# nianticlabs/simplerecon

Measured on AMD Instinct MI355X. Metric: depth frames/sec (640x480, 7 src views, 64 planes), higher is better.
Workload: dtype f32

## Files before the change

### include/simplerecon_hip.h

```cpp
#ifndef SIMPLERECON_HIP_H_
#define SIMPLERECON_HIP_H_

#include <stddef.h>
#include <stdint.h>

#ifdef __cplusplus
extern "C" {
#endif

#define SR_OK 0
#define SR_ERR_INVALID_ARGUMENT 1
#define SR_ERR_UNSUPPORTED 2
#define SR_ERR_WORKSPACE_TOO_SMALL 3
#define SR_ERR_HIP_BASE 1000

enum {
  SR_OPT_MLP_SPLIT = 0, SR_OPT_WINO_SPLIT, SR_OPT_WINO_XCD, SR_OPT_WINO_NT, SR_OPT_WINO_KSPLIT, SR_OPT_CONV_WINO,
  SR_OPT_CONV_TILE, SR_OPT_CONV_KSPLIT, SR_OPT_PW_NT, SR_OPT_PW_KS, SR_OPT_PT_CFG, SR_OPT_PT_KS, SR_OPT_DOT_LDS,
  SR_OPT_DOT_LDS_G, SR_OPT_DOT_LDS_CULL, SR_OPT_DOT_LDS_CAP, SR_OPT_UPSAMPLE_QUAD, SR_OPT_POOL_STREAM,
  SR_OPT_MLP_TILE,
  SR_OPT_COUNT
};
int sr_option_count(void);
const char* sr_option_name(int id);
// ... 128 lines not shown
                              int64_t out_batch_stride, int out_pix_stride, int B, int H, int W, int Cin,
                              int Cout, int ksize, int stride, float leaky_slope, void* workspace,
                              size_t workspace_bytes, void* stream);

size_t sr_wino_packed_weight_floats(int Cout, int Cin);
int sr_wino_pack_weights(const float* weight, int Cout, int Cin, float* packed, void* stream);
int sr_conv_prefers_wino(int B, int H, int W, int Cin, int Cout, int ksize, int stride);
int sr_conv3x3_wino_nhwc_fwd(const float* in, int64_t in_batch_stride, int in_pix_stride,
                             const float* packed_u, const float* bias, const float* residual,
                             int64_t res_batch_stride, int res_pix_stride, float* out,
                             int64_t out_batch_stride, int out_pix_stride, int B, int H, int W, int Cin,
                             int Cout, float leaky_slope, void* stream);

size_t sr_wino4_packed_weight_floats(int Cout, int Cin);
int sr_wino4_pack_weights(const float* weight, int Cout, int Cin, float* packed, void* stream);
int sr_conv_prefers_wino4(int B, int H, int W, int Cin, int Cout, int mode);
int sr_conv3x3_wino4_nhwc_fwd(const float* in, int64_t in_batch_stride, int in_pix_stride, const float* packed_u,
                              const float* bias, const float* residual, int64_t res_batch_stride, int res_pix_stride,
                              float* out, int64_t out_batch_stride, int out_pix_stride, int B, int H, int W, int Cin,
                              int Cout, float leaky_slope, void* stream);

int sr_conv3x3_wino4_variant_nhwc_fwd(const float* in, int64_t in_batch_stride, int in_pix_stride, const float* packed_u,
                                      const float* bias, const float* residual, int64_t res_batch_stride,
                                      int res_pix_stride, float* out, int64_t out_batch_stride, int out_pix_stride, int B,
                                      int H, int W, int Cin, int Cout, float leaky_slope, int variant, void* stream);

int sr_wino_splitk_factor(int B, int H, int W, int Cin, int Cout);
size_t sr_wino_splitk_workspace_bytes(int B, int H, int W, int Cin, int Cout);
int sr_conv3x3_wino_splitk_nhwc_fwd(const float* in, int64_t in_batch_stride, int in_pix_stride,
                                    const float* packed_u, const float* bias, const float* residual,
                                    int64_t res_batch_stride, int res_pix_stride, float* out,
                                    int64_t out_batch_stride, int out_pix_stride, int B, int H, int W, int Cin,
                                    int Cout, float leaky_slope, void* workspace, size_t workspace_bytes,
                                    void* stream);

int sr_wino_conv_plan(int B, int H, int W, int Cin, int Cout, int allow_split, int* nt, int* ks);

int sr_last_launch(char* name, int name_capacity, double* executed_flops);

int sr_upsample2x_nhwc_fwd(const float* in, int64_t in_batch_stride, int in_pix_stride, float* out,
                           int64_t out_batch_stride, int out_pix_stride, int B, int H, int W, int C,
                           void* stream);

int sr_exp_fwd(const float* in, float* out, int64_t n, void* stream);


size_t sr_stem_packed_weight_floats(int Cout);
int sr_stem_pack_weights(const float* weight, int Cout, float* packed, void* stream);

int sr_stem7x7_fwd(const float* in, int64_t in_batch_stride, int64_t in_chan_stride, int64_t in_row_stride,
                   int64_t in_col_stride, const float* packed_weight, const float* scale, const float* shift,
                   float leaky_slope, float* out, int64_t out_batch_stride, int out_pix_stride, int B, int H, int W,
                   int Cout, void* stream);

int sr_maxblurpool_nhwc_fwd(const float* in, int64_t in_batch_stride, int in_pix_stride, float* out,
                            int64_t out_batch_stride, int out_pix_stride, int B, int H, int W, int C, void* stream);

size_t sr_instance_norm_workspace_bytes(int B, int H, int W, int C);
int sr_instance_norm_nhwc_fwd(const float* in, int64_t in_batch_stride, int in_pix_stride, float* out,
                              int64_t out_batch_stride, int out_pix_stride, int B, int H, int W, int C, float eps,
                              float leaky_slope, void* workspace, size_t workspace_bytes, void* stream);

int sr_instance_norm_stats_nhwc(const float* in, int64_t in_batch_stride, int in_pix_stride, int B, int H, int W, int C,
                                float eps, float* stats, void* workspace, size_t workspace_bytes, void* stream);

size_t sr_conv1x1_stats_workspace_bytes(int B, int H, int W, int Cout);
int sr_conv1x1_stats_nhwc_fwd(const float* in, int64_t in_batch_stride, int in_pix_stride, const float* weight,
                              const float* bias, float* out, int64_t out_batch_stride, int out_pix_stride, int B, int H,
                              int W, int Cin, int Cout, float eps, float* stats, void* workspace, size_t workspace_bytes,
                              void* stream);

size_t sr_conv3x3_c16_packed_weight_floats(int Cout, int Cin);
int sr_conv3x3_c16_pack_weights(const float* weight, int Cout, int Cin, float* packed, void* stream);
int sr_conv3x3_c16_nhwc_fwd(const float* in, int64_t in_batch_stride, int in_pix_stride, const float* in_stats,
                            float in_leaky_slope, const float* packed_weight, const float* bias, float* out,
                            int64_t out_batch_stride, int out_pix_stride, int B, int H, int W, int Cin, int Cout,
                            int replicate, float leaky_slope, void* stream);

int sr_tsdf_integrate_fwd(void* tsdf_values, void* tsdf_weights, const void* voxel_coords, int X, int Y, int Z,
                          float origin_x, float origin_y, float origin_z, float voxel_size, const void* depth,
                          const uint8_t* depth_mask, const void* K, const void* T, int B, int H, int W,
                          float min_depth, float max_depth, float depth_range, float truncation, float maxW,
                          void* stream);

size_t sr_mesh_count_scratch_bytes(int X, int Y, int Z);
size_t sr_mesh_list_scratch_bytes(int64_t active);
int sr_mesh_count(const void* tsdf_values, int X, int Y, int Z, float level, void* count_scratch,
                  size_t count_scratch_bytes, int64_t* totals, void* stream);
int sr_mesh_emit(const void* tsdf_values, int X, int Y, int Z, float level, float origin_x, float origin_y, float origin_z,
                 float scale, const void* count_scratch, size_t count_scratch_bytes, void* list_scratch,
                 size_t list_scratch_bytes, int64_t active, int64_t num_vertices, int64_t num_faces, float* vertices,
                 float* normals, int* faces, void* stream);

#define SR_PC_FRAME_FLOATS 36
int sr_pc_consistency(const float* depth, const float* frame_consts, int N, int h, int w, int ref_begin, int ref_count,
                      float z_thresh, float* points, int* counts, void* stream);
int sr_pc_voxel_keys(const float* points, int64_t M, double min_x, double min_y, double min_z, double voxel_size,
                     int64_t* keys, void* stream);
int sr_pc_voxel_mean(const float* points, const uint8_t* colors, int64_t M, const int64_t* order,
                     const int64_t* seg_start, int64_t S, float* out_points, uint8_t* out_colors, void* stream);

#define SR_LOSS_MAX_SOURCES 15
size_t sr_normals_workspace_bytes(int B, int h, int w);
int sr_normals_fwd(const float* depth, const float* invK, int B, int h, int w, float* normals, void* scratch,
                   size_t scratch_bytes, void* stream);
int sr_normals_bwd(const float* grad_normals, const float* depth, const float* invK, int B, int h, int w,
// ... 323 lines not shown
```

### simplerecon_amd/_lib.py

```python
import contextlib
import ctypes as C
import os

import torch

_HERE = os.path.dirname(os.path.abspath(__file__))
LIB_PATH = os.environ.get("SR_HIP_LIBRARY") or os.path.join(_HERE, "libsimplerecon_hip.so")
ABI_VERSION = 4

_lib = None

_p = C.c_void_p
_i = C.c_int
_i64 = C.c_int64
_f = C.c_float
_sz = C.c_size_t

SIGNATURES = {
    "sr_abi_version": (_i, []),
    "sr_option_count": (_i, []),
    "sr_option_name": (C.c_char_p, [_i]),
    "sr_option_id": (_i, [C.c_char_p]),
    "sr_option_get": (_i, [_i, C.POINTER(C.c_int)]),
    "sr_option_set": (_i, [_i, _i, C.POINTER(C.c_int)]),
# ... 71 lines not shown
    "sr_act_bwd": (_i, [_p, _p, _p, _i64, _f, _p]),
    "sr_act_bwd_bias_workspace_bytes": (_sz, [_i64, _i]),
    "sr_act_bwd_bias_nhwc": (_i, [_p, _p, _p, _p, _i64, _i, _f, _p, _sz, _p]),
    "sr_zero_stuff2x_nhwc": (_i, [_p, _i64, _i, _p, _i, _i, _i, _i, _i, _i, _p]),
    "sr_upsample2x_bwd_nhwc": (_i, [_p, _i64, _i, _p, _i64, _i, _i, _i, _i, _i, _p]),
    "sr_conv_flip_transpose_weights": (_i, [_p, _i, _i, _i, _p, _p]),
    "sr_mul_fwd": (_i, [_p, _p, _p, _i64, _p]),
    "sr_norm_workspace_bytes": (_sz, [_i, _i, _i, _i]),
    "sr_norm_stats_nhwc": (_i, [_p, _i64, _i, _i, _i, _i, _i, _p, _p, _p, _sz, _p]),
    "sr_norm_act_fwd_nhwc": (_i, [_p, _i64, _i, _p, _p, _f, _p, _p, _f, _i, _p, _i64, _i, _i, _i, _i, _p]),
    "sr_norm_act_bwd_nhwc": (_i, [_p, _i64, _i, _p, _i64, _i, _p, _p, _f, _p, _p, _f, _i, _i, _p, _i64, _i, _p, _p,
                                  _i, _i, _i, _p, _sz, _p]),
    "sr_rowsum_nhwc": (_i, [_p, _i64, _i, _p, _i64, _i, _i, _i, _i, _f, _p, _p, _sz, _p]),
    "sr_maxblurpool_bwd_workspace_bytes": (_sz, [_i, _i, _i, _i]),
    "sr_maxblurpool_bwd_nhwc": (_i, [_p, _i64, _i, _p, _i64, _i, _p, _i64, _i, _i, _i, _i, _i, _p, _sz, _p]),
    "sr_replicate_pad_nhwc_fwd": (_i, [_p, _i64, _i, _p, _i, _i, _i, _i, _i, _p]),
    "sr_replicate_pad_nhwc_bwd": (_i, [_p, _p, _i, _i, _i, _i, _i, _p]),
    "sr_im2col7x7s2_nhwc": (_i, [_p, _i64, _i64, _i64, _i64, _p, _i, _i, _i, _i, _p]),
    "sr_dwconv3x3_bwd_workspace_bytes": (_sz, [_i, _i, _i, _i]),
    "sr_dwconv3x3_bwd_nhwc": (_i, [_p, _i64, _i, _p, _i64, _i, _p, _p, _p, _i, _i, _i, _i, _i, _i, _i, _i, _i, _p, _sz,
                                   _p]),
    "sr_scale_bwd_nhwc": (_i, [_p, _i64, _i, _p, _p, _f, _p, _i, _i, _i, _p]),
    "sr_small_linear_fwd": (_i, [_p, _p, _p, _p, _p, _i, _i, _i, _f, _p]),
    "sr_small_linear_bwd": (_i, [_p, _p, _p, _p, _p, _p, _p, _i, _i, _i, _f, _p]),
    "sr_act_in_bwd": (_i, [_p, _p, _p, _i64, _f, _p]),
    "sr_add_act_fwd": (_i, [_p, _p, _p, _p, _i64, _f, _p]),
    "sr_conv_wgrad_padded_workspace_bytes": (_sz, [_i, _i, _i, _i, _i, _i]),
    "sr_conv_wgrad_padded_nhwc": (_i, [_p, _i64, _i, _p, _i64, _i, _p, _i, _i, _i, _i, _i, _i, _i, _i, _i, _i, _i, _p,
                                       _sz, _p]),
    "sr_conv_splitk_workspace_bytes": (_sz, [_i, _i, _i, _i, _i, _i, _i]),
    "sr_conv2d_splitk_nhwc_fwd": (_i, [_p, _i64, _i, _p, _p, _p, _i64, _i, _p, _i64, _i, _i, _i, _i, _i, _i, _i, _i,
                                       _f, _p, _sz, _p]),
    "sr_wino_packed_weight_floats": (_sz, [_i, _i]),
    "sr_wino_pack_weights": (_i, [_p, _i, _i, _p, _p]),
    "sr_conv_prefers_wino": (_i, [_i, _i, _i, _i, _i, _i, _i]),
    "sr_wino_splitk_factor": (_i, [_i, _i, _i, _i, _i]),
    "sr_wino_splitk_workspace_bytes": (_sz, [_i, _i, _i, _i, _i]),
    "sr_conv3x3_wino_splitk_nhwc_fwd": (_i, [_p, _i64, _i, _p, _p, _p, _i64, _i, _p, _i64, _i, _i, _i, _i, _i, _i, _f,
                                             _p, _sz, _p]),
    "sr_wino_conv_plan": (_i, [_i, _i, _i, _i, _i, _i, _p, _p]),
    "sr_last_launch": (_i, [_p, _i, _p]),
    "sr_conv3x3_wino_nhwc_fwd": (_i, [_p, _i64, _i, _p, _p, _p, _i64, _i, _p, _i64, _i, _i, _i, _i, _i, _i, _f, _p]),
    "sr_wino4_packed_weight_floats": (_sz, [_i, _i]),
    "sr_wino4_pack_weights": (_i, [_p, _i, _i, _p, _p]),
    "sr_conv_prefers_wino4": (_i, [_i, _i, _i, _i, _i, _i]),
    "sr_conv3x3_wino4_nhwc_fwd": (_i, [_p, _i64, _i, _p, _p, _p, _i64, _i, _p, _i64, _i, _i, _i, _i, _i, _i, _f, _p]),
    "sr_conv3x3_wino4_variant_nhwc_fwd": (_i, [_p, _i64, _i, _p, _p, _p, _i64, _i, _p, _i64, _i, _i, _i, _i, _i, _i, _f, _i,
                                               _p]),
    "sr_upsample2x_nhwc_fwd": (_i, [_p, _i64, _i, _p, _i64, _i, _i, _i, _i, _i, _p]),
    "sr_exp_fwd": (_i, [_p, _p, _i64, _p]),
    "sr_stem_packed_weight_floats": (_sz, [_i]),
    "sr_stem_pack_weights": (_i, [_p, _i, _p, _p]),
    "sr_stem7x7_fwd": (_i, [_p, _i64, _i64, _i64, _i64, _p, _p, _p, _f, _p, _i64, _i, _i, _i, _i, _i, _p]),
    "sr_maxblurpool_nhwc_fwd": (_i, [_p, _i64, _i, _p, _i64, _i, _i, _i, _i, _i, _p]),
    "sr_instance_norm_workspace_bytes": (_sz, [_i, _i, _i, _i]),
    "sr_instance_norm_nhwc_fwd": (_i, [_p, _i64, _i, _p, _i64, _i, _i, _i, _i, _i, _f, _f, _p, _sz, _p]),
    "sr_instance_norm_stats_nhwc": (_i, [_p, _i64, _i, _i, _i, _i, _i, _f, _p, _p, _sz, _p]),
    "sr_conv1x1_stats_workspace_bytes": (_sz, [_i, _i, _i, _i]),
    "sr_conv1x1_stats_nhwc_fwd": (_i, [_p, _i64, _i, _p, _p, _p, _i64, _i, _i, _i, _i, _i, _i, _f, _p, _p, _sz, _p]),
    "sr_conv3x3_c16_packed_weight_floats": (_sz, [_i, _i]),
    "sr_conv3x3_c16_pack_weights": (_i, [_p, _i, _i, _p, _p]),
    "sr_conv3x3_c16_nhwc_fwd": (_i, [_p, _i64, _i, _p, _f, _p, _p, _p, _i64, _i, _i, _i, _i, _i, _i, _i, _f, _p]),
    "sr_tsdf_integrate_fwd": (_i, [_p, _p, _p, _i, _i, _i, _f, _f, _f, _f, _p, _p, _p, _p, _i, _i, _i,
                                   _f, _f, _f, _f, _f, _p]),
    "sr_mesh_count_scratch_bytes": (_sz, [_i, _i, _i]),
    "sr_mesh_list_scratch_bytes": (_sz, [_i64]),
    "sr_mesh_count": (_i, [_p, _i, _i, _i, _f, _p, _sz, _p, _p]),
    "sr_mesh_emit": (_i, [_p, _i, _i, _i, _f, _f, _f, _f, _f, _p, _sz, _p, _sz, _i64, _i64, _i64, _p, _p, _p, _p]),
    "sr_pc_consistency": (_i, [_p, _p, _i, _i, _i, _i, _i, _f, _p, _p, _p]),
    "sr_pc_voxel_keys": (_i, [_p, _i64, C.c_double, C.c_double, C.c_double, C.c_double, _p, _p]),
    "sr_pc_voxel_mean": (_i, [_p, _p, _i64, _p, _p, _i64, _p, _p, _p]),
    "sr_normals_workspace_bytes": (_sz, [_i, _i, _i]),
    "sr_normals_fwd": (_i, [_p, _p, _i, _i, _i, _p, _p, _sz, _p]),
    "sr_normals_bwd": (_i, [_p, _p, _p, _i, _i, _i, _p, _p, _sz, _p]),
    "sr_normals_loss_workspace_bytes": (_sz, [_i, _i, _i]),
    "sr_normals_loss_fwd": (_i, [_p, _p, _i, _i, _i, _p, _p, _sz, _p]),
    "sr_normals_loss_bwd": (_i, [_p, _p, _p, _p, _i, _i, _i, _p, _p]),
    "sr_grad_loss_workspace_bytes": (_sz, [_i, _i, _i]),
    "sr_grad_loss_fwd": (_i, [_p, _p, _i, _i, _i, _p, _p, _sz, _p]),
    "sr_grad_loss_bwd": (_i, [_p, _p, _p, _p, _i, _i, _i, _p, _p, _sz, _p]),
    "sr_mv_loss_workspace_bytes": (_sz, [_i, _i, _i, _i]),
    "sr_mv_loss_fwd": (_i, [_p, _p, _p, _p, _p, _p, _p, _i, _i, _i, _i, _f, _p, _p, _p, _p, _sz, _p]),
    "sr_mv_loss_bwd": (_i, [_p, _p, _p, _p, _p, _p, _p, _p, _p, _i, _i, _i, _i, _f, _p, _p]),
    "sr_depth_terms_workspace_bytes": (_sz, [_i, _i, _i]),
    "sr_depth_terms_fwd": (_i, [_p, _p, _p, _p, _p, _i, _i, _p, _i, _i, _p, _i, _i, _i, _i, _i, _f, _i, _p, _p, _sz,
                                _p]),
    "sr_depth_terms_bwd": (_i, [_p, _p, _p, _p, _p, _p, _p, _i, _i, _p, _i, _i, _p, _i, _i, _i, _i, _i, _f, _i, _p, _p,
                                _p, _p, _p, _p]),
    "sr_depth_metrics_workspace_bytes": (_sz, [_i, _i, _i]),
    "sr_depth_metrics": (_i, [_p, _p, _p, _f, _i, _i, _i, _i, _i, _i, _i, _p, _p, _p, _p, _sz, _p]),
    "sr_depth_metrics_gather": (_i, [_p, _i, _i, _i, _i, _i, _i, _p, _p]),
    "sr_nn_grid_plan": (_i, [_i64, _p, _i64, _p, _p, _p]),
    "sr_nn_keys": (_i, [_p, _i64, C.c_double, C.c_double, C.c_double, C.c_double, _i, _i, _i, _p, _p]),
    "sr_nn_build": (_i, [_p, _i64, _p, _p, _i64, _p, _p, _p]),
    "sr_nn_query": (_i, [_p, _i64, _p, _p, _i64, _p, _i64, C.c_double, C.c_double, C.c_double, C.c_double, _i, _i, _i,
                         _p, _p, _p, _p]),
    "sr_sample_surface_workspace_bytes": (_sz, [_i64]),
    "sr_sample_surface_cdf": (_i, [_p, _i64, _p, _i64, _p, _p, _sz, _p]),
    "sr_sample_surface": (_i, [_p, _i64, _p, _i64, _p, _i64, C.c_uint64, _p, _p, _p]),
    "sr_mesh_metrics_workspace_bytes": (_sz, [_i64, _i64]),
    "sr_mesh_metrics": (_i, [_p, _i64, _p, _i64, _f, _p, _p, _sz, _p]),
    "sr_stsdf_touch": (_i, [_p, _i, _i, _i, _p, C.c_double, C.c_double, _p, _p]),
    "sr_stsdf_block_masks": (_i, [_p, _p, _i64, _i64, _p, _p]),
    "sr_stsdf_integrate": (_i, [_p, _i64, _p, _p, _p, _i64, _p, _p, _p, _i, _i, _i, _f, _f, _p]),
    "sr_stsdf_mesh_count": (_i, [_p, _i64, _p, _p, _i64, _p, _p]),
    "sr_stsdf_mesh_emit": (_i, [_p, _i64, _p, _p, _i64, _f, _p, _i64, _i64, _p, _p, _p, _p, _p]),
# ... 221 lines not shown
```

### simplerecon_amd/csrc/sr_matching.hip

```cpp
#include "sr_common.h"

typedef float v16f __attribute__((ext_vector_type(16)));
#define SR_MFMA(a, b, c) __builtin_amdgcn_mfma_f32_32x32x2f32((a), (b), (c), 0, 0, 0)

#define SR_STEM_T 16
#define SR_STEM_PR 37
#define SR_STEM_PW 37
#define SR_STEM_STEPS 74
#define SR_STEM_WFLOATS (SR_STEM_STEPS * 128)
#define SR_STEM_PFLOATS (3 * SR_STEM_PR * SR_STEM_PW)

struct SrStemParams {
  const float* in; int64_t sb, sc, sy, sx;
  const float* wp;
  const float* scale; const float* shift;
  float slope;
  float* out; int64_t out_sb; int out_sp;
  int H, W, Ho, Wo, tiles_x, tiles_y, total;
};

__global__ void sr_stem_pack_kernel(const float* __restrict__ w , float* __restrict__ packed) {
  for (int idx = blockIdx.x * blockDim.x + threadIdx.x; idx < SR_STEM_WFLOATS; idx += gridDim.x * blockDim.x) {
    const int step = idx >> 7, r = idx & 127;
    const int half = r >> 6, col = (r & 63) >> 1, nt = r & 1;
    const int tap = 2 * step + half;
    const int co = nt * 32 + col;
    packed[idx] = tap < 147 ? w[co * 147 + tap] : 0.f;
  }
}

__host__ __device__ constexpr int sr_stem_tap_offset(int k) {
  return k >= 147 ? 0 : ((k / 49) * SR_STEM_PR + (k % 49) / 7) * SR_STEM_PW + (k % 7);
}

__global__ __launch_bounds__(256, 2) void sr_stem_kernel(SrStemParams p) {
  __shared__ __attribute__((aligned(16))) float wl[SR_STEM_WFLOATS];
  __shared__ float patch[SR_STEM_PFLOATS];
  const int lane = threadIdx.x & 63, wave = threadIdx.x >> 6;
  const int i = lane & 31, half = lane >> 5;

  for (int e = threadIdx.x; e < SR_STEM_WFLOATS / 4; e += 256)
    reinterpret_cast<float4*>(wl)[e] = reinterpret_cast<const float4*>(p.wp)[e];

  int abase[2];
#pragma unroll
  for (int m = 0; m < 2; ++m) abase[m] = (2 * (4 * wave + 2 * m + (i >> 4))) * SR_STEM_PW + 2 * (i & 15);
  const float2* wl2 = reinterpret_cast<const float2*>(wl) + half * 32 + i;

  float sc[2], sh[2];
#pragma unroll
  for (int n = 0; n < 2; ++n) {
    sc[n] = p.scale ? p.scale[n * 32 + i] : 1.f;
    sh[n] = p.shift ? p.shift[n * 32 + i] : 0.f;
  }

  constexpr int PF = (SR_STEM_PFLOATS + 255) / 256;
  float pf[PF];
  auto fetch = [&](int tile) {
    const int tx = tile % p.tiles_x, ty = (tile / p.tiles_x) % p.tiles_y, b = tile / (p.tiles_x * p.tiles_y);
    const float* __restrict__ img = p.in + (int64_t)b * p.sb;
#pragma unroll
    for (int it = 0; it < PF; ++it) {
      const int e = threadIdx.x + it * 256;
      const int c = e / (SR_STEM_PR * SR_STEM_PW), rem = e - c * (SR_STEM_PR * SR_STEM_PW);
      const int r = rem / SR_STEM_PW, x = rem - r * SR_STEM_PW;
      const int gy = 2 * ty * SR_STEM_T - 3 + r, gx = 2 * tx * SR_STEM_T - 3 + x;
      const bool ok = (e < SR_STEM_PFLOATS) & (gy >= 0) & (gy < p.H) & (gx >= 0) & (gx < p.W);
      const int64_t off = ok ? c * p.sc + gy * p.sy + gx * p.sx : 0;
      const float v = img[off];
      pf[it] = ok ? v : 0.f;
    }
  };
  auto stash = [&]() {
#pragma unroll
    for (int it = 0; it < PF; ++it) {
      const int e = threadIdx.x + it * 256;
      if (e < SR_STEM_PFLOATS) patch[e] = pf[it];
    }
  };
  if ((int)blockIdx.x < p.total) fetch(blockIdx.x);
  stash();
  __syncthreads();

  for (int tile = blockIdx.x; tile < p.total; tile += gridDim.x) {
    const int tx = tile % p.tiles_x, ty = (tile / p.tiles_x) % p.tiles_y, b = tile / (p.tiles_x * p.tiles_y);
    const int oy0 = ty * SR_STEM_T, ox0 = tx * SR_STEM_T;
    const int next = tile + gridDim.x;
    if (next < p.total) fetch(next);
    __builtin_amdgcn_sched_barrier(0);

    v16f acc[2][2];
#pragma unroll
    for (int m = 0; m < 2; ++m)
#pragma unroll
      for (int n = 0; n < 2; ++n)
#pragma unroll
        for (int r = 0; r < 16; ++r) acc[m][n][r] = 0.f;

#pragma unroll
    for (int step = 0; step < SR_STEM_STEPS; ++step) {
      constexpr int dummy = 0; (void)dummy;
      const int o0 = sr_stem_tap_offset(2 * step), o1 = sr_stem_tap_offset(2 * step + 1);
      const int oa = (o1 == o0 + 1) ? o0 + half : (half ? o1 : o0);
      const float a0 = patch[abase[0] + oa], a1 = patch[abase[1] + oa];
      const float2 w = wl2[step * 64];
      acc[0][0] = SR_MFMA(a0, w.x, acc[0][0]);
      acc[1][0] = SR_MFMA(a1, w.x, acc[1][0]);
      acc[0][1] = SR_MFMA(a0, w.y, acc[0][1]);
      acc[1][1] = SR_MFMA(a1, w.y, acc[1][1]);
    }
    __builtin_amdgcn_sched_barrier(0);
    __syncthreads();
    if (next < p.total) stash();
    __syncthreads();

    float* __restrict__ ob = p.out + (int64_t)b * p.out_sb;
#pragma unroll
    for (int m = 0; m < 2; ++m)
#pragma unroll
      for (int r = 0; r < 16; ++r) {
        const int mrow = (r & 3) + 8 * (r >> 2) + 4 * half;
        const int oy = oy0 + 4 * wave + 2 * m + (mrow >> 4), ox = ox0 + (mrow & 15);
        if (oy < p.Ho && ox < p.Wo) {
          float* o = ob + ((int64_t)oy * p.Wo + ox) * p.out_sp + i;
#pragma unroll
          for (int n = 0; n < 2; ++n) {
            float v = acc[m][n][r] * sc[n] + sh[n];
            if (p.slope >= 0.f) v = v >= 0.f ? v : v * p.slope;
            o[n * 32] = v;
          }
        }
      }
  }
}

__device__ __forceinline__ int sr_reflect(int i, int n) { return i < 0 ? -i : (i >= n ? 2 * n - 2 - i : i); }
__device__ __forceinline__ float sr_nanmax(float a, float b) { return (a > b || a != a) ? a : b; }
__device__ __forceinline__ float4 sr_max4(float4 a, float4 b) {
  return make_float4(sr_nanmax(a.x, b.x), sr_nanmax(a.y, b.y), sr_nanmax(a.z, b.z), sr_nanmax(a.w, b.w));
}
__device__ __forceinline__ float4 sr_axpy4(float s, float4 a, float4 acc) {
  return make_float4(acc.x + s * a.x, acc.y + s * a.y, acc.z + s * a.z, acc.w + s * a.w);
}

__device__ __forceinline__ float4 sr_ld4(const float* p) { return *reinterpret_cast<const float4*>(p); }

__device__ __forceinline__ float4 sr_maxblur_generic(const float* __restrict__ ib, int in_sp, int W, int Hm, int Wm,
                                                     int oy, int ox, int c4) {
  const float f[4] = {0.125f, 0.375f, 0.375f, 0.125f};
  float4 acc = make_float4(0.f, 0.f, 0.f, 0.f);
  for (int i = 0; i < 4; ++i) {
    const int my = sr_reflect(2 * oy - 1 + i, Hm);
    float4 row = make_float4(0.f, 0.f, 0.f, 0.f);
    for (int j = 0; j < 4; ++j) {
      const int mx = sr_reflect(2 * ox - 1 + j, Wm);
      const float* q = ib + ((int64_t)my * W + mx) * in_sp + 4 * c4;
      row = sr_axpy4(f[j], sr_max4(sr_max4(sr_ld4(q), sr_ld4(q + in_sp)),
                                   sr_max4(sr_ld4(q + (int64_t)W * in_sp), sr_ld4(q + (int64_t)W * in_sp + in_sp))), row);
    }
    acc = sr_axpy4(f[i], row, acc);
  }
  return acc;
}

__global__ __launch_bounds__(256) void sr_maxblurpool_kernel(const float* __restrict__ in, int64_t in_sb, int in_sp,
                                                             float* __restrict__ out, int64_t out_sb, int out_sp,
                                                             int H, int W, int Ho, int Wo, int C4, int xcd_order) {
  constexpr int BW = 2;
  constexpr int WC = 2 * BW + 3;
  const int Hm = H - 1, Wm = W - 1;
  const int bx = (Wo + BW - 1) / BW, by = (Ho + 1) / 2;
  const int64_t total = (int64_t)bx * by * C4;
  const float f[4] = {0.125f, 0.375f, 0.375f, 0.125f};
  unsigned bxi = blockIdx.x, byi = blockIdx.y;
  if (xcd_order) {
    const unsigned T = gridDim.x * gridDim.y, L = blockIdx.y * gridDim.x + blockIdx.x;
    const unsigned Lp = (L & 7u) * (T >> 3) + (L >> 3);
    byi = Lp / gridDim.x;
    bxi = Lp - byi * gridDim.x;
  }
  const float* __restrict__ ib = in + (int64_t)byi * in_sb;
  float* __restrict__ ob = out + (int64_t)byi * out_sb;
  for (int64_t idx = (int64_t)bxi * blockDim.x + threadIdx.x; idx < total; idx += (int64_t)gridDim.x * blockDim.x) {
    const int c4 = (int)(idx % C4);
    const int blk = (int)(idx / C4);
    const int oy0 = 2 * (blk / bx), ox0 = BW * (blk % bx);
// ... 535 lines not shown

extern "C" size_t sr_conv3x3_c16_packed_weight_floats(int Cout, int Cin) {
  if (Cout <= 0 || Cout > 16 || Cin <= 0 || (Cin % 32)) return 0;
  return (size_t)(Cin / 32) * 9 * 2 * 64 * 4;
}

extern "C" int sr_conv3x3_c16_pack_weights(const float* weight, int Cout, int Cin, float* packed, void* stream_) {
  if (!weight || !packed) return SR_ERR_INVALID_ARGUMENT;
  if (Cout <= 0 || Cout > 16 || Cin <= 0 || (Cin % 32)) return SR_ERR_UNSUPPORTED;
  hipLaunchKernelGGL(sr_t16_pack_kernel, dim3(64), dim3(256), 0, (hipStream_t)stream_, weight, packed, Cout, Cin);
  return sr_hip_rc(hipGetLastError());
}

extern "C" int sr_conv3x3_c16_nhwc_fwd(const float* in, int64_t in_batch_stride, int in_pix_stride,
                                       const float* in_stats, float in_leaky_slope, const float* packed_weight,
                                       const float* bias, float* out, int64_t out_batch_stride, int out_pix_stride,
                                       int B, int H, int W, int Cin, int Cout, int replicate, float leaky_slope,
                                       void* stream_) {
  if (B < 0 || H <= 0 || W <= 0 || Cin <= 0 || Cout <= 0) return SR_ERR_INVALID_ARGUMENT;
  if (B == 0) return SR_OK;
  if (!in || !packed_weight || !out) return SR_ERR_INVALID_ARGUMENT;
  if (Cout > 16 || (Cin % 32) || (in_pix_stride % 4) || (in_batch_stride % 4) || ((uintptr_t)in & 15) ||
      (in_stats && ((uintptr_t)in_stats & 15)))
    return SR_ERR_UNSUPPORTED;
  SrT16Params p;
  p.in = in; p.in_sb = in_batch_stride; p.in_sp = in_pix_stride;
  p.stats = in_stats; p.in_slope = in_leaky_slope;
  p.wp = packed_weight; p.bias = bias;
  p.out = out; p.out_sb = out_batch_stride; p.out_sp = out_pix_stride;
  p.H = H; p.W = W; p.Cin = Cin; p.Cout = Cout; p.replicate = replicate;
  p.tiles_x = (W + 15) / 16; p.tiles_y = (H + 7) / 8;
  p.total = p.tiles_x * p.tiles_y * B;
  p.out_slope = leaky_slope;
  int blocks = 3 * sr_cus();
  if (blocks > p.total) blocks = p.total;
  const bool norm = in_stats != nullptr, act = in_leaky_slope >= 0.f;
  sr_note_launch({SR_K_T16, 0, 0, 0, 0, 0, 0, (int64_t)p.total * ((SR_T16_HH - 2) * (SR_T16_HW - 2)), 16, (int64_t)Cin * 9});
  if (norm && act) hipLaunchKernelGGL((sr_t16_kernel<true, true>), dim3(blocks), dim3(256), 0, (hipStream_t)stream_, p);
  else if (norm) hipLaunchKernelGGL((sr_t16_kernel<true, false>), dim3(blocks), dim3(256), 0, (hipStream_t)stream_, p);
  else if (act) hipLaunchKernelGGL((sr_t16_kernel<false, true>), dim3(blocks), dim3(256), 0, (hipStream_t)stream_, p);
  else hipLaunchKernelGGL((sr_t16_kernel<false, false>), dim3(blocks), dim3(256), 0, (hipStream_t)stream_, p);
  return sr_hip_rc(hipGetLastError());
}

extern "C" size_t sr_stem_packed_weight_floats(int Cout) { return Cout == 64 ? (size_t)SR_STEM_WFLOATS : 0; }

extern "C" int sr_stem_pack_weights(const float* weight, int Cout, float* packed, void* stream_) {
  if (!weight || !packed) return SR_ERR_INVALID_ARGUMENT;
  if (Cout != 64) return SR_ERR_UNSUPPORTED;
  hipLaunchKernelGGL(sr_stem_pack_kernel, dim3(42), dim3(256), 0, (hipStream_t)stream_, weight, packed);
  return sr_hip_rc(hipGetLastError());
}

extern "C" int sr_stem7x7_fwd(const float* in, int64_t in_batch_stride, int64_t in_chan_stride, int64_t in_row_stride,
                              int64_t in_col_stride, const float* packed_weight, const float* scale,
                              const float* shift, float leaky_slope, float* out, int64_t out_batch_stride,
                              int out_pix_stride, int B, int H, int W, int Cout, void* stream_) {
  if (B < 0 || H <= 0 || W <= 0) return SR_ERR_INVALID_ARGUMENT;
  if (Cout != 64) return SR_ERR_UNSUPPORTED;
  if (B == 0) return SR_OK;
  if (!in || !packed_weight || !out) return SR_ERR_INVALID_ARGUMENT;
  SrStemParams p;
  p.in = in; p.sb = in_batch_stride; p.sc = in_chan_stride; p.sy = in_row_stride; p.sx = in_col_stride;
  p.wp = packed_weight; p.scale = scale; p.shift = shift; p.slope = leaky_slope;
  p.out = out; p.out_sb = out_batch_stride; p.out_sp = out_pix_stride;
  p.H = H; p.W = W;
  p.Ho = (H + 6 - 7) / 2 + 1; p.Wo = (W + 6 - 7) / 2 + 1;
  p.tiles_x = (p.Wo + SR_STEM_T - 1) / SR_STEM_T; p.tiles_y = (p.Ho + SR_STEM_T - 1) / SR_STEM_T;
  p.total = p.tiles_x * p.tiles_y * B;
  int blocks = 2 * sr_cus();
  if (blocks > p.total) blocks = p.total;
  sr_note_launch({SR_K_STEM, 0, 0, 0, 0, 0, 0, (int64_t)p.total * (SR_STEM_T * SR_STEM_T), 64, 2 * SR_STEM_STEPS});
  hipLaunchKernelGGL(sr_stem_kernel, dim3(blocks), dim3(256), 0, (hipStream_t)stream_, p);
  return sr_hip_rc(hipGetLastError());
}

extern "C" int sr_maxblurpool_nhwc_fwd(const float* in, int64_t in_batch_stride, int in_pix_stride, float* out,
                                       int64_t out_batch_stride, int out_pix_stride, int B, int H, int W, int C,
                                       void* stream_) {
  if (B < 0 || H < 4 || W < 4 || C <= 0) return SR_ERR_INVALID_ARGUMENT;
  if (B == 0) return SR_OK;
  if (!in || !out) return SR_ERR_INVALID_ARGUMENT;
  if ((C % 4) || (in_pix_stride % 4) || (out_pix_stride % 4) || (in_batch_stride % 4) || (out_batch_stride % 4) ||
      ((uintptr_t)in & 15) || ((uintptr_t)out & 15))
    return SR_ERR_UNSUPPORTED;
  const int Ho = (H - 2) / 2 + 1, Wo = (W - 2) / 2 + 1;
  if (sr_opt(SR_OPT_POOL_STREAM) && H >= 16 && W >= 16 && B <= 65535) {
    SrPoolStreamParams p;
    p.in = in; p.in_sb = in_batch_stride; p.in_sp = in_pix_stride;
    p.out = out; p.out_sb = out_batch_stride; p.out_sp = out_pix_stride;
    p.H = H; p.W = W; p.Ho = Ho; p.Wo = Wo; p.C4 = C / 4;
    p.oy_lo = 1; p.oy_hi = (H - 4) / 2; p.ox_lo = 1; p.ox_hi = (W - 4) / 2;
    const int rows = p.oy_hi - p.oy_lo + 1, cols = p.ox_hi - p.ox_lo + 1;
    p.col_blocks = (cols + 1) / 2;
    p.col_groups = (int)(((int64_t)p.col_blocks * p.C4 + 255) / 256);
    const int slots = 2 * sr_cus(), per_band = B * p.col_groups;
    int best_bands = 1;
    double best = -1.0;
    for (int nb = 1; nb <= (rows >= 8 ? rows / 8 : 1); ++nb) {
      const int br = (rows + nb - 1) / nb, real = (rows + br - 1) / br;
      const int64_t wgs = (int64_t)real * per_band;
      const int64_t rounds = (wgs + slots - 1) / slots;
      if (rounds > 10 && best >= 0.0) break;
      const double eff = (double)wgs / (double)(rounds * slots) * (2.0 * br) / (2.0 * br + 3.0);
      if (eff > best + 1e-9) { best = eff; best_bands = real; }
    }
    p.band_rows = (rows + best_bands - 1) / best_bands;
    p.bands = (rows + p.band_rows - 1) / p.band_rows;
    p.stream_wgs = p.bands * p.col_groups;
    p.frame_rows_top = p.oy_lo; p.frame_rows_bottom = Ho - 1 - p.oy_hi;
    p.frame_cols_left = p.ox_lo; p.frame_cols_right = Wo - 1 - p.ox_hi;
    const int64_t frame = ((int64_t)(p.frame_rows_top + p.frame_rows_bottom) * Wo +
                           (int64_t)rows * (p.frame_cols_left + p.frame_cols_right)) * p.C4;
    int frame_wgs = (int)((frame + 255) / 256 < 1024 ? (frame + 255) / 256 : 1024);
    hipLaunchKernelGGL(sr_maxblurpool_stream_kernel, dim3(p.stream_wgs + frame_wgs, B), dim3(256), 0, (hipStream_t)stream_, p);
    return sr_hip_rc(hipGetLastError());
  }
  const int64_t total = (int64_t)((Ho + 1) / 2) * ((Wo + 1) / 2) * (C / 4);
  const int blocks = (int)((total + 255) / 256 < 8192 ? (total + 255) / 256 : 8192);
  const int xcd = ((int64_t)blocks * 256 >= total) && (((int64_t)blocks * B) % 8 == 0);
  hipLaunchKernelGGL(sr_maxblurpool_kernel, dim3(blocks, B), dim3(256), 0, (hipStream_t)stream_, in, in_batch_stride,
                     in_pix_stride, out, out_batch_stride, out_pix_stride, H, W, Ho, Wo, C / 4, xcd);
  return sr_hip_rc(hipGetLastError());
}

static void sr_inorm_chunks(int B, int HW, int* chunks, int* chunk_pix) {
  int want = (8 * sr_cus() + B - 1) / B;
// ... 102 lines not shown
```

Baseline: 329.2.

## Add lean stem 7x7 kernel with prefetched patches and buffer loads

Adds a new path for the 7x7 stem conv that walks tiles persistently. It prefetches the next tile's input patch into registers through buffer loads while the MFMA loop runs on the current tile. Precomputed per-thread offsets, interior-tile fast paths and templated activation/scale variants cut address arithmetic and bounds checks. Bounds-checked buffer stores handle edge tiles. It becomes the default when the strides fit 32-bit buffer ranges, at the cost of more registers and a more complex kernel.

```diff
diff --git a/include/simplerecon_hip.h b/include/simplerecon_hip.h
--- a/include/simplerecon_hip.h
+++ b/include/simplerecon_hip.h
@@ -204,6 +204,11 @@
                    int64_t in_col_stride, const float* packed_weight, const float* scale, const float* shift,
                    float leaky_slope, float* out, int64_t out_batch_stride, int out_pix_stride, int B, int H, int W,
                    int Cout, void* stream);
+
+int sr_stem7x7_variant_fwd(const float* in, int64_t in_batch_stride, int64_t in_chan_stride, int64_t in_row_stride,
+                           int64_t in_col_stride, const float* packed_weight, const float* scale, const float* shift,
+                           float leaky_slope, float* out, int64_t out_batch_stride, int out_pix_stride, int B, int H, int W,
+                           int Cout, int variant, void* stream);
 
 int sr_maxblurpool_nhwc_fwd(const float* in, int64_t in_batch_stride, int in_pix_stride, float* out,
                             int64_t out_batch_stride, int out_pix_stride, int B, int H, int W, int C, void* stream);
diff --git a/simplerecon_amd/_lib.py b/simplerecon_amd/_lib.py
--- a/simplerecon_amd/_lib.py
+++ b/simplerecon_amd/_lib.py
@@ -147,6 +147,7 @@
     "sr_stem_packed_weight_floats": (_sz, [_i]),
     "sr_stem_pack_weights": (_i, [_p, _i, _p, _p]),
     "sr_stem7x7_fwd": (_i, [_p, _i64, _i64, _i64, _i64, _p, _p, _p, _f, _p, _i64, _i, _i, _i, _i, _i, _p]),
+    "sr_stem7x7_variant_fwd": (_i, [_p, _i64, _i64, _i64, _i64, _p, _p, _p, _f, _p, _i64, _i, _i, _i, _i, _i, _i, _p]),
     "sr_maxblurpool_nhwc_fwd": (_i, [_p, _i64, _i, _p, _i64, _i, _i, _i, _i, _i, _p]),
     "sr_instance_norm_workspace_bytes": (_sz, [_i, _i, _i, _i]),
     "sr_instance_norm_nhwc_fwd": (_i, [_p, _i64, _i, _p, _i64, _i, _i, _i, _i, _i, _f, _f, _p, _sz, _p]),
diff --git a/simplerecon_amd/csrc/sr_matching.hip b/simplerecon_amd/csrc/sr_matching.hip
--- a/simplerecon_amd/csrc/sr_matching.hip
+++ b/simplerecon_amd/csrc/sr_matching.hip
@@ -1,4 +1,8 @@
+#include <type_traits>
+
 #include "sr_common.h"
+#include "sr_buffer.h"
+#include "sr_view.h"
 
 typedef float v16f __attribute__((ext_vector_type(16)));
 #define SR_MFMA(a, b, c) __builtin_amdgcn_mfma_f32_32x32x2f32((a), (b), (c), 0, 0, 0)
@@ -17,6 +21,7 @@
   float slope;
   float* out; int64_t out_sb; int out_sp;
   int H, W, Ho, Wo, tiles_x, tiles_y, total;
+  int64_t in_span, out_span;
 };
 
 __global__ void sr_stem_pack_kernel(const float* __restrict__ w , float* __restrict__ packed) {
@@ -33,9 +38,7 @@
   return k >= 147 ? 0 : ((k / 49) * SR_STEM_PR + (k % 49) / 7) * SR_STEM_PW + (k % 7);
 }
 
-__global__ __launch_bounds__(256, 2) void sr_stem_kernel(SrStemParams p) {
-  __shared__ __attribute__((aligned(16))) float wl[SR_STEM_WFLOATS];
-  __shared__ float patch[SR_STEM_PFLOATS];
+__device__ __forceinline__ void sr_stem_tiles_ref(const SrStemParams& p, float* wl, float* patch) {
   const int lane = threadIdx.x & 63, wave = threadIdx.x >> 6;
   const int i = lane & 31, half = lane >> 5;
 
@@ -132,6 +135,153 @@
         }
       }
   }
+}
+
+#define SR_STEM_PF ((SR_STEM_PFLOATS + 255) / 256)
+struct SrStemTile { int tx, ty, b; };
+
+template <bool ACT, bool SCALE>
+__device__ __forceinline__ void sr_stem_tiles_lean(const SrStemParams& p, float* wl, float* patch ) {
+  constexpr int PF = SR_STEM_PF;
+  const int tid = threadIdx.x, lane = tid & 63, wave = __builtin_amdgcn_readfirstlane(tid >> 6);
+  const int i = lane & 31, half = lane >> 5;
+
+  for (int e = tid; e < SR_STEM_WFLOATS / 4; e += 256)
+    reinterpret_cast<float4*>(wl)[e] = reinterpret_cast<const float4*>(p.wp)[e];
+
+  int abase[2];
+#pragma unroll
+  for (int m = 0; m < 2; ++m) abase[m] = (2 * (4 * wave + 2 * m + (i >> 4))) * SR_STEM_PW + 2 * (i & 15);
+  const float2* wl2 = reinterpret_cast<const float2*>(wl) + half * 32 + i;
+
+  float sc[2], sh[2];
+#pragma unroll
+  for (int n = 0; n < 2; ++n) {
+    sc[n] = SCALE ? p.scale[n * 32 + i] : 1.f;
+    sh[n] = p.shift ? p.shift[n * 32 + i] : 0.f;
+  }
+
+  unsigned roff[PF], rx[PF];
+#pragma unroll
+  for (int it = 0; it < PF; ++it) {
+    const int e = tid + it * 256;
+    const int c = e / (SR_STEM_PR * SR_STEM_PW), rem = e - c * (SR_STEM_PR * SR_STEM_PW);
+    const int r = rem / SR_STEM_PW, x = rem - r * SR_STEM_PW;
+    roff[it] = e < SR_STEM_PFLOATS ? (unsigned)(uint64_t)(c * p.sc + r * p.sy + x * p.sx) * 4u : SR_OOB;
+    rx[it] = (unsigned)r | ((unsigned)x << 8);
+  }
+
+  const int G = gridDim.x;
+  const SrStemTile step = {G % p.tiles_x, (G / p.tiles_x) % p.tiles_y, G / (p.tiles_x * p.tiles_y)};
+  auto advance = [&](SrStemTile t) {
+    t.tx += step.tx;
+    if (t.tx >= p.tiles_x) { t.tx -= p.tiles_x; ++t.ty; }
+    t.ty += step.ty;
+    if (t.ty >= p.tiles_y) { t.ty -= p.tiles_y; ++t.b; }
+    t.b += step.b;
+    return t;
+  };
+  auto interior = [&](SrStemTile t) -> bool {
+    return (t.ty >= 1) & (2 * t.ty * SR_STEM_T + SR_STEM_PR - 4 < p.H) & (t.tx >= 1) & (2 * t.tx * SR_STEM_T + SR_STEM_PW - 4 < p.W);
+  };
+
+  float pf[PF];
+  auto fetch = [&](SrStemTile t, bool live, bool inside) {
+    const int gy0 = 2 * t.ty * SR_STEM_T - 3, gx0 = 2 * t.tx * SR_STEM_T - 3;
+    const int64_t origin = gy0 * p.sy + gx0 * p.sx;
+    int64_t bytes = live ? p.in_span - 4 * origin : 0;
+    if (bytes > 0x7fffffff) bytes = 0x7fffffff;
+    const __amdgpu_buffer_rsrc_t rs = sr_rsrc(p.in + (live ? t.b * p.sb + origin : 0), bytes);
+    unsigned vo[PF];
+    if (inside) {
+#pragma unroll
+      for (int it = 0; it < PF; ++it) vo[it] = roff[it];
+    } else {
+#pragma unroll
+      for (int it = 0; it < PF; ++it) {
+        const bool ok = ((unsigned)(gy0 + (int)(rx[it] & 255u)) < (unsigned)p.H) & ((unsigned)(gx0 + (int)(rx[it] >> 8)) < (unsigned)p.W);
+        vo[it] = ok ? roff[it] : SR_OOB;
+      }
+    }
+#pragma unroll
+    for (int it = 0; it < PF; ++it)
+      pf[it] = __builtin_bit_cast(float, __builtin_amdgcn_raw_buffer_load_b32(rs, (int)vo[it], 0, 0));
+  };
+  auto stash = [&]() {
+#pragma unroll
+    for (int it = 0; it < PF; ++it) patch[tid + it * 256] = pf[it];
+  };
+
+  const unsigned lane_off = (unsigned)(4 * half * p.out_sp + i) * 4u;
+  const unsigned row_bytes = (unsigned)p.Wo * (unsigned)p.out_sp * 4u, pix_bytes = (unsigned)p.out_sp * 4u;
+
+  int tile = blockIdx.x;
+  SrStemTile cur = {tile % p.tiles_x, (tile / p.tiles_x) % p.tiles_y, tile / (p.tiles_x * p.tiles_y)};
+  bool cur_inside = interior(cur);
+  fetch(cur, tile < p.total, cur_inside);
+  stash();
+  __syncthreads();
+
+  for (; tile < p.total; tile += G) {
+    const SrStemTile nxt = advance(cur);
+    const bool nxt_inside = interior(nxt);
+    fetch(nxt, tile + G < p.total, nxt_inside);
+    __builtin_amdgcn_sched_barrier(0);
+
+    v16f acc[2][2];
+    const v16f zero = {0.f, 0.f, 0.f, 0.f, 0.f, 0.f, 0.f, 0.f, 0.f, 0.f, 0.f, 0.f, 0.f, 0.f, 0.f, 0.f};
+#pragma unroll
+    for (int step_k = 0; step_k < SR_STEM_STEPS; ++step_k) {
+      const int o0 = sr_stem_tap_offset(2 * step_k), o1 = sr_stem_tap_offset(2 * step_k + 1);
+      const int oa = (o1 == o0 + 1) ? o0 + half : (half ? o1 : o0);
+      const float a0 = patch[abase[0] + oa], a1 = patch[abase[1] + oa];
+      const float2 w = wl2[step_k * 64];
+      acc[0][0] = SR_MFMA(a0, w.x, step_k ? acc[0][0] : zero);
+      acc[1][0] = SR_MFMA(a1, w.x, step_k ? acc[1][0] : zero);
+      acc[0][1] = SR_MFMA(a0, w.y, step_k ? acc[0][1] : zero);
+      acc[1][1] = SR_MFMA(a1, w.y, step_k ? acc[1][1] : zero);
+    }
+    __builtin_amdgcn_sched_barrier(0);
+    __syncthreads();
+    stash();
+    __syncthreads();
+
+    const int oy0 = cur.ty * SR_STEM_T + 4 * wave, ox0 = cur.tx * SR_STEM_T;
+    const int64_t first = ((int64_t)oy0 * p.Wo + ox0) * p.out_sp;
+    int64_t obytes = p.out_span - 4 * first;
+    if (obytes < 0) obytes = 0;
+    const __amdgpu_buffer_rsrc_t os = sr_rsrc(p.out + cur.b * p.out_sb + first, obytes);
+    const int ylim = p.Ho - oy0, xlim = p.Wo - ox0;
+    auto store_tile = [&](auto border) {
+#pragma unroll
+      for (int m = 0; m < 2; ++m)
+#pragma unroll
+        for (int r = 0; r < 16; ++r) {
+          const int dy = 2 * m + (r >> 3), dx = (r & 3) + 8 * ((r >> 2) & 1);
+          const unsigned delta = (unsigned)dy * row_bytes + (unsigned)dx * pix_bytes;
+          unsigned vo = lane_off;
+          if (decltype(border)::value) vo = (4 * half < (dy < ylim ? xlim - dx : 0)) ? lane_off : SR_OOB;
+#pragma unroll
+          for (int n = 0; n < 2; ++n) {
+            float v = SCALE ? __builtin_fmaf(acc[m][n][r], sc[n], sh[n]) : acc[m][n][r] + sh[n];
+            if (ACT) v = v >= 0.f ? v : v * p.slope;
+            __builtin_amdgcn_raw_buffer_store_b32(__builtin_bit_cast(unsigned, v), os, (int)(vo + n * 128u), (int)delta, 0);
+          }
+        }
+    };
+    if (cur_inside) store_tile(std::false_type{});
+    else store_tile(std::true_type{});
+    cur = nxt;
+    cur_inside = nxt_inside;
+  }
+}
+
+template <int FORM, bool ACT, bool SCALE>
+__global__ __launch_bounds__(256, 2) void sr_stem_kernel(SrStemParams p) {
+  __shared__ __attribute__((aligned(16))) float wl[SR_STEM_WFLOATS];
+  __shared__ float patch[FORM ? SR_STEM_PF * 256 : SR_STEM_PFLOATS];
+  if (FORM == 0) sr_stem_tiles_ref(p, wl, patch);
+  else sr_stem_tiles_lean<ACT, SCALE>(p, wl, patch);
 }
 
 __device__ __forceinline__ int sr_reflect(int i, int n) { return i < 0 ? -i : (i >= n ? 2 * n - 2 - i : i); }
@@ -773,10 +923,10 @@
   return sr_hip_rc(hipGetLastError());
 }
 
-extern "C" int sr_stem7x7_fwd(const float* in, int64_t in_batch_stride, int64_t in_chan_stride, int64_t in_row_stride,
-                              int64_t in_col_stride, const float* packed_weight, const float* scale,
-                              const float* shift, float leaky_slope, float* out, int64_t out_batch_stride,
-                              int out_pix_stride, int B, int H, int W, int Cout, void* stream_) {
+static int sr_stem_run(const float* in, int64_t in_batch_stride, int64_t in_chan_stride, int64_t in_row_stride,
+                       int64_t in_col_stride, const float* packed_weight, const float* scale, const float* shift,
+                       float leaky_slope, float* out, int64_t out_batch_stride, int out_pix_stride, int B, int H, int W,
+                       int Cout, int variant, void* stream_) {
   if (B < 0 || H <= 0 || W <= 0) return SR_ERR_INVALID_ARGUMENT;
   if (Cout != 64) return SR_ERR_UNSUPPORTED;
   if (B == 0) return SR_OK;
@@ -789,11 +939,43 @@
   p.Ho = (H + 6 - 7) / 2 + 1; p.Wo = (W + 6 - 7) / 2 + 1;
   p.tiles_x = (p.Wo + SR_STEM_T - 1) / SR_STEM_T; p.tiles_y = (p.Ho + SR_STEM_T - 1) / SR_STEM_T;
   p.total = p.tiles_x * p.tiles_y * B;
+  const int64_t lim = (int64_t)1 << 29;
+  const bool strides_ok = in_chan_stride >= 0 && in_row_stride >= 0 && in_col_stride >= 0 && in_chan_stride < lim &&
+                          in_row_stride < lim && in_col_stride < lim && out_pix_stride >= 64;
+  p.in_span = strides_ok ? (2 * in_chan_stride + (H - 1) * in_row_stride + (W - 1) * in_col_stride + 1) * 4 : -1;
+  p.out_span = strides_ok ? sr_view_span((int64_t)p.Ho * p.Wo, out_pix_stride, 64, 4) : -1;
+  const bool fits = strides_ok && sr_span_fits32(p.in_span + 12 * (in_row_stride + in_col_stride)) && sr_span_fits32(p.out_span);
+  if (variant == 2 && !fits) return SR_ERR_UNSUPPORTED;
   int blocks = 2 * sr_cus();
   if (blocks > p.total) blocks = p.total;
   sr_note_launch({SR_K_STEM, 0, 0, 0, 0, 0, 0, (int64_t)p.total * (SR_STEM_T * SR_STEM_T), 64, 2 * SR_STEM_STEPS});
-  hipLaunchKernelGGL(sr_stem_kernel, dim3(blocks), dim3(256), 0, (hipStream_t)stream_, p);
+  const bool lean = variant != 1 && fits, act = leaky_slope >= 0.f, affine = scale != nullptr;
+  const dim3 grid(blocks), wg(256);
+  hipStream_t stream = (hipStream_t)stream_;
+  if (!lean) hipLaunchKernelGGL((sr_stem_kernel<0, false, false>), grid, wg, 0, stream, p);
+  else if (act && affine) hipLaunchKernelGGL((sr_stem_kernel<1, true, true>), grid, wg, 0, stream, p);
+  else if (act) hipLaunchKernelGGL((sr_stem_kernel<1, true, false>), grid, wg, 0, stream, p);
+  else if (affine) hipLaunchKernelGGL((sr_stem_kernel<1, false, true>), grid, wg, 0, stream, p);
+  else hipLaunchKernelGGL((sr_stem_kernel<1, false, false>), grid, wg, 0, stream, p);
   return sr_hip_rc(hipGetLastError());
+}
+
+extern "C" int sr_stem7x7_fwd(const float* in, int64_t in_batch_stride, int64_t in_chan_stride, int64_t in_row_stride,
+                              int64_t in_col_stride, const float* packed_weight, const float* scale,
+                              const float* shift, float leaky_slope, float* out, int64_t out_batch_stride,
+                              int out_pix_stride, int B, int H, int W, int Cout, void* stream_) {
+  return sr_stem_run(in, in_batch_stride, in_chan_stride, in_row_stride, in_col_stride, packed_weight, scale, shift,
+                     leaky_slope, out, out_batch_stride, out_pix_stride, B, H, W, Cout, 0, stream_);
+}
+
+extern "C" int sr_stem7x7_variant_fwd(const float* in, int64_t in_batch_stride, int64_t in_chan_stride,
+                                      int64_t in_row_stride, int64_t in_col_stride, const float* packed_weight,
+                                      const float* scale, const float* shift, float leaky_slope, float* out,
+                                      int64_t out_batch_stride, int out_pix_stride, int B, int H, int W, int Cout,
+                                      int variant, void* stream_) {
+  if (variant < 0 || variant > 2) return SR_ERR_INVALID_ARGUMENT;
+  return sr_stem_run(in, in_batch_stride, in_chan_stride, in_row_stride, in_col_stride, packed_weight, scale, shift,
+                     leaky_slope, out, out_batch_stride, out_pix_stride, B, H, W, Cout, variant, stream_);
 }
 
 extern "C" int sr_maxblurpool_nhwc_fwd(const float* in, int64_t in_batch_stride, int in_pix_stride, float* out,
```

New measurement: 331.3, median of 6. About the same (+0.6%).
